# LouisBearing/BirdSoundClassif

Hardware: AMD Instinct MI355X
Metric: clips/sec (3 s @ 22.05 kHz) detect fwd (higher is better)
Workload: dtype f32; 1 GPU; BASELINE.json configs[1]: 1xMI355X inference, batch=64 synthetic 3 s clips (PCM16 @22.05 kHz resident in HBM) through the HIP STFT front end + detector forward + device post-processing, detections returned to the host; batch_per_gpu=64, distinct_clips=64, lanes=2

## Files before the change

birdsoundclassif_amd/_lib.py:

```python
import ctypes as C
import os
import subprocess

_HERE = os.path.dirname(os.path.abspath(__file__))
LIB_PATH = os.environ.get('NBM_LIB') or os.path.join(_HERE, 'libnbm_hip.so')
CSRC = os.path.join(_HERE, 'csrc')

_lib = None


class GemmDesc(C.Structure):
    _fields_ = [('x', C.c_void_p), ('w', C.c_void_p), ('y', C.c_void_p),
                ('scale', C.c_void_p), ('shift', C.c_void_p), ('residual', C.c_void_p),
                ('x_gs', C.c_int64), ('w_gs', C.c_int64), ('y_gs', C.c_int64), ('res_gs', C.c_int64),
                ('groups', C.c_int),
                ('B', C.c_int), ('H', C.c_int), ('W', C.c_int), ('Cin', C.c_int),
                ('N', C.c_int),
                ('kh', C.c_int), ('kw', C.c_int), ('stride', C.c_int), ('pad', C.c_int),
                ('Ho', C.c_int), ('Wo', C.c_int),
                ('x_ld', C.c_int), ('w_ld', C.c_int), ('y_ld', C.c_int), ('res_ld', C.c_int),
                ('alpha', C.c_float), ('act', C.c_int), ('shift_per_row', C.c_int),
                ('up', C.c_void_p), ('up_H', C.c_int), ('up_W', C.c_int),
                ('rows', C.c_void_p), ('rows_blocks', C.c_void_p),
                ('rows_mode', C.c_int), ('rows_count', C.c_int), ('rows_TH', C.c_int), ('rows_TW', C.c_int),
# ... 110 lines not shown
    'nbm_zero_tiles': [_P, _I, _I, _I, _I, _P, _I, _P, _P],
    'nbm_tiles_gather': [_P, _I, _I, _I, _I, _P, _I, _P, _P, _P],
    'nbm_tiles_scatter_add': [_P, _I, _I, _I, _I, _P, _I, _P, _P, _P],
    'nbm_proposal_iou': [_P, _P, _P, _I, _I, _I, _P, _P, _P],
    'nbm_anchor_targets': [_P, _I, _P, _P, _I, _I, _F, _F, _P, _P, _P, _P],
    'nbm_maxpool3x3s2_bwd': [_P, _P, _P, _I, _I, _I, _I, _I, _I, _P, _P, _P],
    'nbm_upsample_bilinear_bwd': [_P, _I, _I, _I, _I, _P, _I, _I, _I, _P],
    'nbm_tiles_upsample_bilinear_bwd_add': [_P, _I, _I, _I, _I, _P, _I, _P, _P, _I, _I, _P],
    'nbm_png_unfilter_gray8': [_P, _L, _I, _I, _I, _P, _L, _P, _P],
    'nbm_image_half_std_u8': [_P, _L, _I, _L, _P, _P],
    'nbm_randn_fill': [_U64, _L, _P, _P],
    'nbm_augment_batch': [_P, _P, _P, _I, _I, _I, _P, _P, _P, _P, _P, _P, _P],
    'nbm_u8_to_unit': [_P, _L, _P, _P],
    'nbm_wino_input': [_P, _I, _I, _I, _I, _P, _I, _P],
    'nbm_wino_output': [_P, _P, _P, _P, _I, _I, _I, _I, _I, _P, _I, _P, _P],
    'nbm_wino_outgrad': [_P, _I, _I, _I, _I, _P, _P, _I, _P],
    'nbm_wino_weight': [_P, _P, _I, _I, _I, _I, _P, _P],
    'nbm_wino_weight_grad': [_P, _P, _I, _I, _I, _P, _P],
    'nbm_wino23_rows': [_P, _I, _I, _I, _I, _P, _P],
    'nbm_wino23_conv_fused': [_P, _P, _P, _P, _P, _I, _I, _I, _I, _I, _I, _P, _I, _P],
    'nbm_wino23_rows_tiles': [_P, _I, _I, _I, _I, _P, _I, _P, _P, _P, _I, _P],
    'nbm_wino23_conv_fused_tiles': [_P, _P, _P, _P, _P, _I, _I, _I, _I, _I, _I, _P, _P, _I, _P, _P, _P],
    'nbm_roi_tiles': [_P, _P, _I, _I, _I, _I, _P, _P, _P, _I, _P, _P, _P],
    'nbm_wino23_input_tiles': [_P, _I, _I, _I, _I, _P, _I, _P, _P, _P],
    'nbm_wino23_outgrad_tiles': [_P, _I, _I, _I, _I, _P, _I, _P, _P, _P, _I, _P],
    'nbm_cell_outgrad': [_P, _I, _I, _I, _I, _I, _P, _P, _P],
    'nbm_cell_weight': [_P, _I, _I, _P, _I, _P, _I, _P],
    'nbm_cell_weight_fold': [_P, _P, _I, _I, _I, _I, _F, _P, _I, _P, _I, _P],
    'nbm_cell_weight_grad': [_P, _I, _I, _I, _P, _P],
    'nbm_cell_input': [_P, _I, _I, _I, _I, _I, _P, _I, _I, _P],
    'nbm_cell_input_up': [_P, _P, _I, _I, _I, _I, _I, _I, _I, _P, _I, _I, _P],
    'nbm_cell_patches': [_P, _I, _I, _I, _I, _I, _P, _I, _I, _P],
    'nbm_cell_patches_up': [_P, _P, _I, _I, _I, _I, _I, _I, _I, _P, _I, _I, _P],
    'nbm_cell_dgrad_output': [_P, _I, _I, _I, _I, _I, _P, _I, _I, _I, _P, _P],
    'nbm_cell_output': [_P, _P, _I, _I, _I, _I, _I, _P, _P],
    'nbm_weighted_sum': [_P, _P, _P, _P, _P, _L, _P],
    'nbm_weighted_sum_bwd': [_P, _P, _P, _P, _P, _P, _P, _P, _P, _L, _P],
    'nbm_softmax_rows_bwd': [_P, _P, _P, _L, _I, _F, _P],
    'nbm_pair_softmax_bwd': [_P, _P, _P, _L, _P],
    'nbm_dwconv3x3_bwd': [_P, _P, _P, _I, _I, _I, _I, _I, _I, _P, _P, _P, _I, _I, _P],
    'nbm_dwconv3x3_bwd_acc': [_P, _P, _I, _I, _I, _I, _I, _I, _P, _I, _I, _P],
    'nbm_film_fwd': [_P, _P, _P, _L, _I, _P],
    'nbm_film_bwd': [_P, _P, _P, _P, _P, _L, _I, _P],
    'nbm_bn_train_fwd': [_P, _L, _I, _P, _P, _F, _F, _P, _P, _P, _P, _P, _P, _P],
    'nbm_bn_train_bwd': [_P, _P, _L, _I, _P, _P, _P, _P, _P, _P, _P, _P],
    'nbm_roi_pool_bwd': [C.POINTER(C.c_void_p), C.POINTER(C.c_int), C.POINTER(C.c_int), _I, _I, _P, _P, _I, _I, _P, _P],
    'nbm_sqnorm_accum': [_P, _L, _P, _P],
    'nbm_adamw_step': [_P, _P, _P, _P, _L, _F, _F, _F, _F, _F, _I, _P, _F, _P],
}


def build(verbose=False):
    r = subprocess.run(['make', '-C', CSRC, '-j4'], capture_output=True, text=True)
    if verbose or r.returncode:
        print(r.stdout[-4000:], r.stderr[-4000:])
    if r.returncode:
        raise RuntimeError('building libnbm_hip.so failed')
    return LIB_PATH


def load():
    global _lib
    if _lib is not None:
        return _lib
    import torch
    if not os.path.isfile(LIB_PATH):
# ... 25 lines not shown
```

birdsoundclassif_amd/csrc/cellwino.hip:

```cpp
#include "nbm_common.h"

namespace {

constexpr int NP = 5;
constexpr int MAX_BIAS_N = 2048;
__device__ constexpr float CE[5][3] = {{1.f, 0.f, 0.f}, {1.f, 1.f, 1.f}, {1.f, -1.f, 1.f}, {1.f, 2.f, 4.f}, {1.f, -2.f, 4.f}};
__device__ constexpr float CV[5][5] = {{1.f, 0.f, 0.f, 0.f, 0.f},
                                       {0.f, 2.f / 3, -2.f / 3, -1.f / 12, 1.f / 12},
                                       {-5.f / 4, 2.f / 3, 2.f / 3, -1.f / 24, -1.f / 24},
                                       {0.f, -1.f / 6, 1.f / 6, 1.f / 12, -1.f / 12},
                                       {1.f / 4, -1.f / 6, -1.f / 6, 1.f / 24, 1.f / 24}};

struct CellGeom { int B, H, W, C4, S, OH, OW; long long T; };

__device__ __forceinline__ void cell_of(const CellGeom& q, unsigned cell, int& b, int& oy, int& ox) {
  ox = (int)(cell % (unsigned)q.OW);
  const unsigned r = cell / (unsigned)q.OW;
  oy = (int)(r % (unsigned)q.OH);
  b = (int)(r / (unsigned)q.OH);
}

__global__ __launch_bounds__(256) void cell_outgrad_kernel(const float* __restrict__ g, const CellGeom q, float* __restrict__ Vg,
                                                           float* __restrict__ bias_grad) {
  const f32x4* g4 = reinterpret_cast<const f32x4*>(g);
// ... 129 lines not shown
        lxs[l] = fminf(fmaxf(fx - x0, 0.f), 1.f);
        v00[l] = s4[((rb + y0) * Wc + x0) * q.C4 + c]; v01[l] = s4[((rb + y0) * Wc + x1i) * q.C4 + c];
        v10[l] = s4[((rb + y1) * Wc + x0) * q.C4 + c]; v11[l] = s4[((rb + y1) * Wc + x1i) * q.C4 + c];
      }
      __builtin_amdgcn_sched_barrier(0);
#pragma unroll
      for (int l = 0; l < NP; ++l) {
        const bool ok = yin && (unsigned)(q.S * ox - 2 + l) < (unsigned)q.W;
        const float lx = lxs[l], hx = 1.f - lx;
        f32x4 v;
#pragma unroll
        for (int e = 0; e < 4; ++e)
          v[e] = ok ? (hy * (hx * v00[l][e] + lx * v01[l][e]) + ly * (hx * v10[l][e] + lx * v11[l][e])) + bv[e] : 0.f;
        if constexpr (RAW) {
          v4[((long long)(j * NP + l) * q.T + cell) * ld4 + coff4 + c] = v;
        } else {
#pragma unroll
          for (int a = 0; a < NP; ++a)
            if (CV[j][a] != 0.f) t[a][l] += CV[j][a] * v;
        }
      }
    }
    if constexpr (RAW) continue;
#pragma unroll
    for (int a = 0; a < NP; ++a)
#pragma unroll
      for (int e = 0; e < NP; ++e) {
        f32x4 o = zero;
#pragma unroll
        for (int l = 0; l < NP; ++l)
          if (CV[l][e] != 0.f) o += CV[l][e] * t[a][l];
        v4[((long long)(a * NP + e) * q.T + cell) * ld4 + coff4 + c] = o;
      }
  }
}

__global__ __launch_bounds__(256) void cell_dgrad_output_kernel(const float* __restrict__ M, const CellGeom q, float* __restrict__ gx,
                                                                int cls, int ld4, int coff4, float* __restrict__ bias_grad) {
  const f32x4* m4 = reinterpret_cast<const f32x4*>(M);
  f32x4* o4 = reinterpret_cast<f32x4*>(gx);
  const f32x4 zero = {0.f, 0.f, 0.f, 0.f};
  f32x4 bsum = zero;
  int my_c = -1;
  const int cy = cls >= 0 ? cls >> 1 : 0, cx = cls >= 0 ? cls & 1 : 0;
  const int OHc = cls >= 0 ? (q.OH - cy + 1) >> 1 : q.OH, OWc = cls >= 0 ? (q.OW - cx + 1) >> 1 : q.OW;
  const unsigned total = (unsigned)((long long)q.B * OHc * OWc * q.C4);
  for (unsigned i = blockIdx.x * 256u + threadIdx.x; i < total; i += gridDim.x * 256u) {
    const int c = (int)(i % (unsigned)q.C4);
    unsigned rest = i / (unsigned)q.C4;
    int ox = (int)(rest % (unsigned)OWc); rest /= (unsigned)OWc;
    int oy = (int)(rest % (unsigned)OHc);
    const int b = (int)(rest / (unsigned)OHc);
    if (cls >= 0) { oy = 2 * oy + cy; ox = 2 * ox + cx; }
    const unsigned cell = ((unsigned)b * q.OH + oy) * q.OW + ox;
    my_c = c;
    f32x4 t[NP][NP];
#pragma unroll
    for (int j = 0; j < NP; ++j)
#pragma unroll
      for (int e = 0; e < NP; ++e) t[j][e] = zero;
#pragma unroll
    for (int a = 0; a < NP; ++a)
#pragma unroll
      for (int e = 0; e < NP; ++e) {
        const f32x4 v = m4[((long long)(a * NP + e) * q.T + cell) * ld4 + coff4 + c];
#pragma unroll
// ... 209 lines not shown
}

extern "C" int nbm_cell_input_up(const float* x1, const float* bias, int B, int H, int W, int C, int Hc, int Wc, int stride, float* Vx,
                                 int ld, int c_off, void* stream) {
  CellGeom q;
  if (!x1 || !Vx || !cell_geom(B, H, W, C, stride, q) || Hc <= 0 || Wc <= 0 || ld < c_off + C || c_off < 0) return NBM_EINVAL;
  if (!nbm_aligned16(x1) || !nbm_aligned16(Vx) || (bias && !nbm_aligned16(bias)) || (ld & 3) || (c_off & 3)) return NBM_EALIGN;
  const float sh = H > 1 ? (float)(Hc - 1) / (float)(H - 1) : 0.f, sw = W > 1 ? (float)(Wc - 1) / (float)(W - 1) : 0.f;
  hipLaunchKernelGGL(cell_input_up_kernel<false>, dim3(stream_grid(q.T * q.C4, q.C4)), dim3(256), 0, (hipStream_t)stream, x1, bias, q, Hc, Wc, sh,
                     sw, Vx, ld / 4, c_off / 4);
  return nbm_launch_status();
}

extern "C" int nbm_cell_patches(const float* x, int B, int H, int W, int C, int stride, float* Vx, int ld, int c_off, void* stream) {
  CellGeom q;
  if (!x || !Vx || !cell_geom(B, H, W, C, stride, q) || ld < c_off + C || c_off < 0) return NBM_EINVAL;
  if (!nbm_aligned16(x) || !nbm_aligned16(Vx) || (ld & 3) || (c_off & 3)) return NBM_EALIGN;
  hipLaunchKernelGGL(cell_input_kernel<true>, dim3(stream_grid(q.T * q.C4, q.C4)), dim3(256), 0, (hipStream_t)stream, x, q, Vx, ld / 4,
                     c_off / 4);
  return nbm_launch_status();
}

extern "C" int nbm_cell_patches_up(const float* x1, const float* bias, int B, int H, int W, int C, int Hc, int Wc, int stride, float* Vx,
                                   int ld, int c_off, void* stream) {
  CellGeom q;
  if (!x1 || !Vx || !cell_geom(B, H, W, C, stride, q) || Hc <= 0 || Wc <= 0 || ld < c_off + C || c_off < 0) return NBM_EINVAL;
  if (!nbm_aligned16(x1) || !nbm_aligned16(Vx) || (bias && !nbm_aligned16(bias)) || (ld & 3) || (c_off & 3)) return NBM_EALIGN;
  const float sh = H > 1 ? (float)(Hc - 1) / (float)(H - 1) : 0.f, sw = W > 1 ? (float)(Wc - 1) / (float)(W - 1) : 0.f;
  hipLaunchKernelGGL(cell_input_up_kernel<true>, dim3(stream_grid(q.T * q.C4, q.C4)), dim3(256), 0, (hipStream_t)stream, x1, bias, q, Hc, Wc,
                     sh, sw, Vx, ld / 4, c_off / 4);
  return nbm_launch_status();
}

extern "C" int nbm_cell_output(const float* M, const float* bias, int B, int H, int W, int N, int stride, float* y, void* stream) {
  CellGeom q;
  if (!M || !y || !cell_geom(B, H, W, N, stride, q)) return NBM_EINVAL;
  if (!nbm_aligned16(M) || !nbm_aligned16(y) || (bias && !nbm_aligned16(bias))) return NBM_EALIGN;
  hipLaunchKernelGGL(cell_output_kernel, dim3(stream_grid(q.T * q.C4, q.C4)), dim3(256), 0, (hipStream_t)stream, M, bias, q, y);
  return nbm_launch_status();
}

extern "C" int nbm_cell_dgrad_output(const float* M, int B, int H, int W, int C, int stride, float* gx, int parity_class, int ld,
                                     int c_off, float* bias_grad, void* stream) {
  CellGeom q;
  if (!M || !gx || parity_class > 3 || !cell_geom(B, H, W, C, stride, q, parity_class < 0 ? 5 : 3)) return NBM_EINVAL;
  if (ld < c_off + C || c_off < 0 || (ld & 3) || (c_off & 3) || (bias_grad && C > MAX_BIAS_N)) return NBM_EINVAL;
  if (!nbm_aligned16(M) || !nbm_aligned16(gx)) return NBM_EALIGN;
  hipLaunchKernelGGL(cell_dgrad_output_kernel, dim3(stream_grid(q.T * q.C4, q.C4)), dim3(256), 0, (hipStream_t)stream, M, q, gx,
                     parity_class, ld / 4, c_off / 4, bias_grad);
  return nbm_launch_status();
}

extern "C" int nbm_cell_weight(const float* w, int N, int C, float* U_nc, int ld, float* U_cn, int ldt, void* stream) {
  if (!w || (!U_nc && !U_cn) || N <= 0 || C <= 0 || (U_nc && ld < C) || (U_cn && ldt < C)) return NBM_EINVAL;
  hipLaunchKernelGGL(cell_weight_kernel, dim3((unsigned)((N * C + 255) / 256)), dim3(256), 0, (hipStream_t)stream, w, N, C, U_nc, ld, U_cn,
                     ldt);
  return nbm_launch_status();
}

extern "C" int nbm_cell_weight_fold(const float* w, const float* w_lat, int wl_ld, int N, int C, int Cin, float alpha, float* U_nc, int ld,
                                    float* U_cn, int ldt, void* stream) {
  if (!w || !w_lat || (!U_nc && !U_cn) || N <= 0 || C <= 0 || Cin <= 0 || wl_ld < Cin || (U_nc && ld < C + Cin) || (U_cn && ldt < C + Cin))
    return NBM_EINVAL;
  hipLaunchKernelGGL(cell_weight_fold_kernel, dim3((unsigned)((N * Cin + 255) / 256)), dim3(256), 0, (hipStream_t)stream, w, w_lat, wl_ld, N,
                     C, Cin, alpha, U_nc, ld, U_cn, ldt);
  return nbm_launch_status();
// ... 38 lines not shown
```

birdsoundclassif_amd/nets/_prep.py:

```python
import weakref

import torch
import torch.nn.functional as F

_cache = {}
_epoch = 0


def bump():
    global _epoch
    _epoch += 1


_DEBUG = __import__('os').environ.get('NBM_PREP_DEBUG') == '1'


def _evict(obj_id):
    for k in [k for k in _cache if k[0] == obj_id]:
        hit = _cache.pop(k, None)
        if _DEBUG and hit is not None:
            v = hit[2]
            ts = [t for t in (v if isinstance(v, (tuple, list)) else [v]) if torch.is_tensor(t)]
            print(f'_prep: evicted {k[1]} (key tensor died), values at {[hex(t.data_ptr()) for t in ts]}', flush=True)

# ... 128 lines not shown
    wp = pt_w.detach().double().reshape(pt_w.shape[0], m_)
    we = torch.einsum('nm,mcae->naec', wp, d)
    const = wp @ cb
    if lat_wk is not None:
        wl = lat_wk.detach().double()
        we = torch.cat([we, float(alpha) * torch.einsum('naec,ci->naei', we, wl)], -1)
    return we, const


def _rpn_extra(out_b, dw_w, dw_b, pt_w, scale, shift, lat_wk, alpha):
    others = [t for t in (out_b, dw_w, dw_b, pt_w, scale, shift, lat_wk) if t is not None]
    return tuple(v for t in others for v in (t.data_ptr(), t._version)) + (float(alpha),)


def rpn_composite(out_w, out_b, dw_w, dw_b, pt_w, scale, shift, lat_wk=None, alpha=1.0, parts=None):
    def make():
        we, const = _rpn_composite64(out_w, out_b, dw_w, dw_b, pt_w, 7, 7, lat_wk, alpha)
        rng = parts if parts is not None else ((0, we.shape[-1]),)
        ws = tuple(we[..., c0:c1].reshape(we.shape[0], -1).float().contiguous() for c0, c1 in rng)
        return ws, scale, (scale.double() * const + shift.double()).float().contiguous()
    return _cached(out_w, ('rpnc', lat_wk is not None, parts), make, extra=_rpn_extra(out_b, dw_w, dw_b, pt_w, scale, shift, lat_wk, alpha))


def rpn_composite_delta(out_w, out_b, dw_w, dw_b, pt_w, scale, shift, rmask, smask, taps, lat_wk=None, alpha=1.0):
    def make():
        we, const = _rpn_composite64(out_w, out_b, dw_w, dw_b, pt_w, rmask, smask, lat_wk, alpha)
        wi, ci = _rpn_composite64(out_w, out_b, dw_w, dw_b, pt_w, 7, 7, lat_wk, alpha)
        d = (we - wi).reshape(we.shape[0], 25, -1)[:, list(taps)] * scale.double()[:, None, None]
        return d.reshape(d.shape[0], -1).float().contiguous(), (scale.double() * (const - ci)).float().contiguous()
    return _cached(out_w, ('rpnd', int(rmask), int(smask), tuple(taps), lat_wk is not None), make,
                   extra=_rpn_extra(out_b, dw_w, dw_b, pt_w, scale, shift, lat_wk, alpha))


def lateral_of_projection(lat_w, lat_b, proj_w, proj_b):
    def make():
        wl = lat_w.detach().double().reshape(lat_w.shape[0], -1)
        wc = wl @ proj_w.detach().double()
        sh = wl @ proj_b.detach().double() + (lat_b.detach().double() if lat_b is not None else 0.0)
        return wc.float().contiguous(), sh.float().contiguous()
    others = [t for t in (lat_b, proj_w, proj_b) if t is not None]
    return _cached(lat_w, 'latproj', make, extra=tuple(v for t in others for v in (t.data_ptr(), t._version)))


def value_of_lateral(lat_w, proj_w, val_w, val_b):
    def make():
        wlo = lat_w.detach().double().reshape(lat_w.shape[0], -1) @ proj_w.detach().double()
        return (wlo @ val_w.detach().double()).float().contiguous(), (wlo @ val_b.detach().double()).float().contiguous()
    others = [proj_w, val_w, val_b]
    return _cached(lat_w, 'vallat', make, extra=tuple(v for t in others for v in (t.data_ptr(), t._version)))


def cat_rows(tag, *tensors):
    def make():
        return torch.cat([t.detach().reshape(t.shape[0], -1) if t.dim() > 1 else t.detach() for t in tensors], 0).contiguous()
    extra = tuple(v for t in tensors for v in (t.data_ptr(), t._version))
    return _cached(tensors[0], ('cat', tag), make, extra=extra)


def clear():
    _cache.clear()
```

birdsoundclassif_amd/ondemand.py:

```python
import ctypes as C
import os
import weakref
from typing import NamedTuple

import numpy as np
import torch

from . import ops
from .ops import check, lib, _ptr, _chk, _stream, gemm_conv, conv_wgrad

LAZY_FINEST = os.environ.get('NBM_LAZY_FINEST', '1') != '0'
COMPOSITE = os.environ.get('NBM_RPN_COMPOSITE', '1') != '0'
TRAIN_COMPOSITE = os.environ.get('NBM_RPN_COMPOSITE_TRAIN', '1') != '0'
LAT_CELL_BWD = os.environ.get('NBM_LAT_CELL_BWD', '1') != '0'
UPBWD_SPLIT = os.environ.get('NBM_UPBWD_SPLIT', '1') != '0'
ZERO_POOL = os.environ.get('NBM_ZERO_POOL', '1') != '0'
ZERO_POOL_CHECK = os.environ.get('NBM_ZERO_POOL_CHECK', '0') == '1'
LAZY_POISON = False
_LAZY = {}
_PATTERNS = {}
_ROI_TILE_BUF = {}


class TilePattern:
    __slots__ = ('tiles', 'blk_info', 'full', 'any', 'n', 'n_eff', 'frac', 'px_rows', 'n_px', 'entry_pm', 'tile_pm')


def wino23_pattern(B, H, W, stride, device, dilate=0):
    key = (B, H, W, stride, str(device), dilate)
    hit = _PATTERNS.get(key)
    if hit is None:
        TH, TW = (H + 1) // 2, (W + 1) // 2

        def need(n, nt):
            m = np.zeros(nt, dtype=np.int64)
            for o in range((n + 2 - 3) // stride + 1):
                for k in range(3):
                    for r in range(o * stride - 1 + k - dilate, o * stride - 1 + k + dilate + 1):
                        if 0 <= r < n:
                            m[r >> 1] |= 1 << (r & 1)
            return m
        ry, rx = need(H, TH), need(W, TW)
        planes_of = {0: 0, 1: 0b0111, 2: 0b1110, 3: 0b1111}

        def plane_mask(cy, cx):
# ... 315 lines not shown
    hit = _BORDER_IDX.get(key)
    if hit is None:
        rm, sm = _tap_masks(H, W, S)
        OH, OW = len(rm), len(sm)
        cls = {}
        for oy in range(OH):
            for ox in range(OW):
                if (rm[oy], sm[ox]) != (7, 7):
                    cls.setdefault((rm[oy], sm[ox]), []).append((oy, ox))
        hit = []
        for (r_, s_), cells in sorted(cls.items()):
            cells = sorted(cells)
            live_a = {a for oy, _ in cells for a in range(5) if 0 <= S * oy - 2 + a < H}
            live_e = {e for _, ox in cells for e in range(5) if 0 <= S * ox - 2 + e < W}
            dropped = [(r, c) for r in range(3) for c in range(3) if not ((r_ >> r) & 1 and (s_ >> c) & 1)]
            taps = [a * 5 + e for a in sorted(live_a) for e in sorted(live_e) if any(0 <= a - r <= 2 and 0 <= e - c <= 2 for r, c in dropped)]
            lin = np.array([oy * OW + ox for oy, ox in cells], dtype=np.int64)
            idx = (np.arange(nb, dtype=np.int64)[:, None] * (OH * OW) + lin[None, :]).reshape(-1)
            py = np.array([[S * oy - 2 + t // 5 for oy, _ in cells] for t in taps], dtype=np.int64)
            px = np.array([[S * ox - 2 + t % 5 for _, ox in cells] for t in taps], dtype=np.int64)
            pix = None
            if taps:
                inside = (py >= 0) & (py < H) & (px >= 0) & (px < W)
                one = np.clip(py, 0, H - 1) * W + np.clip(px, 0, W - 1)
                lin_px = (np.arange(nb, dtype=np.int64)[None, :, None] * (H * W) + one[:, None, :]).reshape(len(taps), -1)
                bad = None if bool(inside.all()) else torch.from_numpy(np.broadcast_to(~inside[:, None, :], (len(taps), nb, len(cells)))
                                                                       .reshape(len(taps), -1).copy()).to(device)
                pix = (torch.from_numpy(lin_px).to(device), bad)
            hit.append((r_, s_, tuple(taps), torch.tensor(taps, dtype=torch.int64, device=device)[:, None], torch.from_numpy(idx).to(device), pix))
        _BORDER_IDX[key] = hit
    return hit


def rpn_composite(fm, block):
    st = lazy_state(fm)
    if st is None or st.pending is None or st.raw is None:
        return None
    from .nets import _prep as prep
    S = st.stride
    if int(max(1, block.stride)) != S or block.stride < 1 or getattr(block, 'pe_proj', None) is not None:
        return None
    B, H, W, _ = fm.shape
    C_ = st.x.shape[-1]
    lt = st.lateral if st.lateral is not None and st.lateral.deferred else None
    Cin = lt.t.shape[-1] if lt is not None else 0
    K = C_ + Cin
    OH, OW = (H - 1) // S + 1, (W - 1) // S + 1
    out_w, out_b = st.raw
    scale, shift = prep.bn_affine(block.norm.weight, block.norm.bias, block.norm.running_mean, block.norm.running_var, block.norm.eps,
                                  conv_bias=block.pt_wise.bias)
    N2 = block.pt_wise.weight.shape[0]
    wargs = (out_w, out_b, block.depth_wise.weight, block.depth_wise.bias, block.pt_wise.weight, scale, shift)
    wkw = dict(lat_wk=lt.wk[:, :Cin] if lt is not None else None, alpha=lt.alpha if lt is not None else 1.0)
    if lt is not None:
        direct_t = Cin % 32 == 0
        operands = [('patch', 0, C_)] + ([('map', lt.t, 0, Cin, C_)] if direct_t else [])
        KV = C_ if direct_t else K
    elif C_ % 32 == 0:
        q32 = C_ // 32
        cc = C_ // (3 if q32 % 3 == 0 else 4 if q32 % 4 == 0 else 2 if q32 % 2 == 0 else 1)
        operands = [('map', st.x, c0, c0 + cc, c0) for c0 in range(0, C_, cc)]
        KV = 0
    else:
        operands, KV = [('patch', 0, C_)], C_
    parts = tuple((0, KV) if op[0] == 'patch' else (op[4], op[4] + op[3] - op[2]) for op in operands)
    ws, sc, sh = prep.rpn_composite(*wargs, **wkw, parts=parts)
    f = torch.empty((B, OH, OW, N2), device=fm.device, dtype=torch.float32)
    stream = _stream()
    keep_label, ops._PROFILE_LABEL = ops._PROFILE_LABEL, ('rpn-composite', H, W)
    try:
        for (b0, nb, pat) in st.chunks:
            T = nb * OH * OW
            V = None
            if KV:
                V = ops._wino_scratch(fm.device, 25 * T * KV, 0)[0]
                if lt is not None:
                    check(lib().nbm_cell_patches_up(_ptr(lt.up[b0:b0 + nb]), _ptr(lt.bias), nb, H, W, C_, lt.up.shape[1], lt.up.shape[2], S,
                                                    _ptr(V), KV, 0, stream), 'nbm_cell_patches_up')
                    if KV > C_:
                        check(lib().nbm_cell_patches(_ptr(lt.t[b0:b0 + nb]), nb, H, W, Cin, S, _ptr(V), KV, C_, stream), 'nbm_cell_patches')
                else:
                    check(lib().nbm_cell_patches(_ptr(st.x[b0:b0 + nb]), nb, H, W, C_, S, _ptr(V), KV, 0, stream), 'nbm_cell_patches')
            fc = f[b0:b0 + nb]
            border = _border_classes(nb, H, W, S, fm.device)
            R = None
            if border:
                R = torch.zeros((T, N2), device=fm.device, dtype=torch.float32)
                Vv = V[:25 * T * KV].view(25, T, KV) if KV else None
                for rmask, smask, taps, tap_idx, idx, pix in border:
                    if not taps:
                        continue
                    dwt, dsh = prep.rpn_composite_delta(*wargs, rmask, smask, taps, **wkw)
                    Tb, nt = idx.numel(), len(taps)
                    cols = []
                    for op in operands:
                        if op[0] == 'patch':
                            cols.append(Vv[tap_idx, idx[None, :]])
                        else:
                            m_ = op[1][b0:b0 + nb]
                            g_ = m_.reshape(-1, m_.shape[-1]).index_select(0, pix[0].reshape(-1))[:, op[2]:op[3]].reshape(nt, Tb, -1)
                            if pix[1] is not None:
                                g_ = g_.masked_fill(pix[1][..., None], 0.0)
                            cols.append(g_)
                    Vb = cols[0] if len(cols) == 1 else torch.cat(cols, -1)
                    fb = torch.empty((Tb, N2), device=fm.device, dtype=torch.float32)
                    if N2 % 32 == 0:
                        gemm_conv(Vb, dwt, fb, B=1, H=nt, W=Tb, Cin=K, N=32, kh=nt, kw=1, Ho=1, Wo=Tb, x_ld=K, w_ld=nt * K, y_ld=N2,
                                  groups=N2 // 32, x_gs=0, w_gs=32 * nt * K, y_gs=32, residual=dsh.expand(Tb, N2).contiguous(), res_ld=N2,
                                  res_gs=32)
                    else:
                        gemm_conv(Vb, dwt, fb, B=1, H=nt, W=Tb, Cin=K, N=N2, kh=nt, kw=1, Ho=1, Wo=Tb, x_ld=K, w_ld=nt * K, shift=dsh)
                    R.index_copy_(0, idx, fb)
            links = []
            for op, w in zip(operands, ws):
                if op[0] == 'patch':
                    ppl = max(1, min(5, ((1 << 31) - (1 << 24)) // (T * KV * 4)))
                    for p0 in range(0, 25, ppl):
                        npl = min(ppl, 25 - p0)
                        links.append(dict(x=V[p0 * T * KV:], w=w[:, p0 * KV:], B=1, H=npl, W=T, Cin=KV, kh=npl, kw=1, Ho=1, Wo=T, x_ld=KV,
                                          w_ld=25 * KV))
                else:
                    m_ = op[1][b0:b0 + nb]
                    cw = op[3] - op[2]
                    links.append(dict(x=m_[..., op[2]:], w=w, B=nb, H=H, W=W, Cin=cw, kh=5, kw=5, stride=S, pad=2, Ho=OH, Wo=OW,
                                      x_ld=m_.shape[-1], w_ld=25 * cw))
            for i, ln in enumerate(links):
                res = R if i == 0 else fc
                ops._PROFILE_LABEL = ('rpn-composite' if ln['kw'] == 1 else 'rpn-composite-map', H, W)
                gemm_conv(ln.pop('x'), ln.pop('w'), fc, N=N2, scale=sc, shift=sh if i == 0 else None, residual=res,
                          res_ld=N2 if res is not None else None, act=ops.ACT_SILU if i == len(links) - 1 else ops.ACT_NONE, **ln)
    finally:
        ops._PROFILE_LABEL = keep_label
    return f


_CE = ((1.0, 0.0, 0.0), (1.0, 1.0, 1.0), (1.0, -1.0, 1.0), (1.0, 2.0, 4.0), (1.0, -2.0, 4.0))


_DEV_CONST = {}


def _dev_const(device, key, values):
    k = (str(device), key)
    t = _DEV_CONST.get(k)
    if t is None:
        t = _DEV_CONST[k] = torch.tensor(values, dtype=torch.float32).to(device)
    return t


def _compose_rpn_cell(dw_w, dw_b, pt_w, pt_b, out_b, masks, mult):
    m_ = dw_w.shape[0]
    n1, n2 = m_ // mult, pt_w.shape[0]
    dev = dw_w.device
    E = _dev_const(dev, 'E', _CE)
    mr = _dev_const(dev, ('rmask', masks), [[float((rm >> r) & 1) for r in range(3)] for rm, _ in masks])
    ms = _dev_const(dev, ('smask', masks), [[float((sm >> c) & 1) for c in range(3)] for _, sm in masks])
    dw = dw_w.reshape(1, m_, 3, 3)
    pt = pt_w.reshape(n2, n1, mult)
    dwm = dw * mr[:, None, :, None] * ms[:, None, None, :]
    t = (E[None, None, :, :, None] * dwm[:, :, None, :, :]).sum(3)
    cw = (t[:, :, :, None, :] * E[None, None, None, :, :]).sum(4)
    cw = cw.reshape(len(masks), n1, mult, 25)
    A = (pt[None, None] * cw.permute(0, 3, 1, 2)[:, :, None]).sum(4)
# ... 596 lines not shown
```

include/nbm_hip.h:

```cpp
#ifndef NBM_HIP_H
#define NBM_HIP_H

#include <stdint.h>

#ifdef __cplusplus
extern "C" {
#endif

#define NBM_OK 0
#define NBM_EINVAL (-1)
#define NBM_EALIGN (-2)
#define NBM_EUNSUPPORTED (-3)

#define NBM_ACT_NONE 0
#define NBM_ACT_RELU 1
#define NBM_ACT_SILU 2
#define NBM_ACT_LEAKY 3

const char* nbm_version(void);

int nbm_graph_census(void* graph, long long counts[6]);

typedef struct nbm_gemm_desc {
  const float* x;
// ... 68 lines not shown
int nbm_wino_weight(const float* g, const float* scale, int N, int C, int transposed, int m, float* U, void* stream);
int nbm_wino_weight_grad(const float* dU, const float* row_scale, int N, int C, int m, float* dW, void* stream);

int nbm_wino23_rows(const float* x, int B, int H, int W, int C, float* R, void* stream);
int nbm_wino23_conv_fused(const float* R, const float* U, const float* scale, const float* shift, const float* mask,
                          int relu, int B, int H, int W, int C, int N, float* y, int variant, void* stream);

int nbm_wino23_rows_tiles(const float* x, int B, int H, int W, int C, const int* tiles, int n_entries, const int* n_blocks,
                          const unsigned* blk_info, float* R,
                          int skip_pattern_stride ,
                          void* stream);
int nbm_wino23_conv_fused_tiles(const float* R, const float* U, const float* scale, const float* shift, const float* mask,
                                int relu ,
                                int B, int H, int W, int C, int N, float* y, const int* tiles, int n_entries,
                                const int* n_blocks, const unsigned* blk_info, void* stream);
int nbm_roi_tiles(const float* rois, const int* n_roi, int B, int roi_cap, int n_levels, int level, const int* fh,
                  const int* fw, const unsigned char* skip, int dilate, int* tiles, int* n_blocks, void* stream);
int nbm_wino23_input_tiles(const float* x, int B, int H, int W, int C, const int* tiles, int n_list, const unsigned* plane_mask,
                           float* V, void* stream);
int nbm_wino23_outgrad_tiles(const float* g, int B, int H, int W, int N, const int* tiles, int n_list, const unsigned* plane_mask,
                             float* dM, float* bias_grad, int skip_pattern_stride, void* stream);
int nbm_cell_outgrad(const float* g, int B, int H, int W, int N, int stride, float* Vg, float* bias_grad, void* stream);
int nbm_cell_weight(const float* w, int N, int C, float* U_nc, int ld, float* U_cn, int ldt, void* stream);
int nbm_cell_weight_fold(const float* w, const float* w_lat, int wl_ld, int N, int C, int Cin, float alpha, float* U_nc, int ld,
                         float* U_cn, int ldt, void* stream);
int nbm_cell_weight_grad(const float* dU, int N, int C, int ld, float* dW, void* stream);
int nbm_cell_input(const float* x, int B, int H, int W, int C, int stride, float* Vx, int ld ,
                   int c_off , void* stream);
int nbm_cell_input_up(const float* x1, const float* bias, int B, int H, int W, int C, int Hc, int Wc, int stride, float* Vx, int ld,
                      int c_off, void* stream);
int nbm_cell_patches(const float* x, int B, int H, int W, int C, int stride, float* Vx, int ld, int c_off, void* stream);
int nbm_cell_patches_up(const float* x1, const float* bias, int B, int H, int W, int C, int Hc, int Wc, int stride, float* Vx, int ld,
                        int c_off, void* stream);

int nbm_copy_rect(float* strided, float* packed, int64_t n_outer, int64_t outer_pitch, int n_rows, int64_t row_pitch, int64_t width,
                  int to_strided, int zero_strided, void* stream);
int nbm_cell_dgrad_output(const float* M, int B, int H, int W, int C, int stride, float* gx, int parity_class,
                          int ld , int c_off ,
                          float* bias_grad , void* stream);
int nbm_cell_output(const float* M, const float* bias, int B, int H, int W, int N, int stride, float* y, void* stream);


int nbm_pcm16_to_wave(const int16_t* pcm, int64_t pcm_ld, int batch, int n, int upsample,
                      const int32_t* hq, int64_t first, int64_t count, float* out, int64_t out_ld, int lead,
                      int pad_mode, void* stream);

int nbm_resample_to_wave(const float* x, int64_t x_ld, int batch, int64_t n, int L, int M, const double* taps, int T,
                         int64_t first, int64_t count, float* out, int64_t out_ld, int lead, int pad_mode, int quant16,
                         void* stream);

#define NBM_WAV_MAX_CHANNELS 8
int nbm_wav_decode(const void* raw, int64_t raw_pitch, int batch, int tag, int bits, int channels, int64_t n, float* out,
                   int64_t out_pitch, void* stream);

int nbm_minmax_init(uint32_t* minmax, int batch, void* stream);
int nbm_stft_db(const float* wave, int64_t wave_ld, int batch, int n_frames, int hop, int n_fft,
                const double* basis, int basis_bin_tiles, int basis_ksteps, int n_bins, float floor_amp,
                float* db, int64_t db_bs, int db_ld, uint32_t* minmax, void* stream);

int nbm_spec_windows(const float* db, int64_t db_bs, int db_ld, int batch, int n_bins, int n_frames,
                     const uint32_t* minmax, float* img, int n_img, int w_pix, int hop_img,
                     const int32_t* last_cols, void* stream);

typedef struct nbm_window_entry {
  const float* db;
  const uint32_t* minmax;
// ... 220 lines not shown
```

Measured before the change: 1073 clips/s.

## Fold horizontal bilinear upsample into RPN composite weights per output column

Adds a column-folded path for the RPN composite conv on upsampled lateral features. The horizontal bilinear interpolation is folded into per-output-column weights, so the new kernel only interpolates vertically and gathers 4 source columns instead of 5 interpolated taps, and the GEMM runs grouped per column with K=5*4*C. This is meant to cut patch-expansion memory traffic and GEMM depth, at the cost of per-column weight tensors (cached), more border-handling code and extra grouped GEMM launches for border rows.

```diff
diff --git a/birdsoundclassif_amd/_lib.py b/birdsoundclassif_amd/_lib.py
--- a/birdsoundclassif_amd/_lib.py
+++ b/birdsoundclassif_amd/_lib.py
@@ -166,6 +166,7 @@
     'nbm_cell_input_up': [_P, _P, _I, _I, _I, _I, _I, _I, _I, _P, _I, _I, _P],
     'nbm_cell_patches': [_P, _I, _I, _I, _I, _I, _P, _I, _I, _P],
     'nbm_cell_patches_up': [_P, _P, _I, _I, _I, _I, _I, _I, _I, _P, _I, _I, _P],
+    'nbm_cell_patches_up_cols': [_P, _P, _I, _I, _I, _I, _I, _I, _I, _P, _P],
     'nbm_cell_dgrad_output': [_P, _I, _I, _I, _I, _I, _P, _I, _I, _I, _P, _P],
     'nbm_cell_output': [_P, _P, _I, _I, _I, _I, _I, _P, _P],
     'nbm_weighted_sum': [_P, _P, _P, _P, _P, _L, _P],
diff --git a/birdsoundclassif_amd/csrc/cellwino.hip b/birdsoundclassif_amd/csrc/cellwino.hip
--- a/birdsoundclassif_amd/csrc/cellwino.hip
+++ b/birdsoundclassif_amd/csrc/cellwino.hip
@@ -185,6 +185,72 @@
           if (CV[l][e] != 0.f) o += CV[l][e] * t[a][l];
         v4[((long long)(a * NP + e) * q.T + cell) * ld4 + coff4 + c] = o;
       }
+  }
+}
+
+__host__ __device__ inline int cell_col_window(int ox, int S, int W, int Wc, float sw, unsigned& used) {
+#pragma clang fp contract(off)
+  int xb = 0x7fffffff, x0s[NP];
+  for (int l = 0; l < NP; ++l) {
+    const int xx = S * ox - 2 + l;
+    const int xc = xx < 0 ? 0 : (xx > W - 1 ? W - 1 : xx);
+    const float fx = sw * xc;
+    x0s[l] = (int)fx;
+    if ((unsigned)xx < (unsigned)W && x0s[l] < xb) xb = x0s[l];
+  }
+  used = 0u;
+  for (int l = 0; l < NP; ++l)
+    if ((unsigned)(S * ox - 2 + l) < (unsigned)W) {
+      const int d0 = x0s[l] - xb, d1 = d0 + (x0s[l] < Wc - 1 ? 1 : 0);
+      used |= (1u << (d0 < 31 ? d0 : 31)) | (1u << (d1 < 31 ? d1 : 31));
+    }
+  return xb;
+}
+
+__global__ __launch_bounds__(256) void cell_patches_up_cols_kernel(const float* __restrict__ x1, const float* __restrict__ bias,
+                                                                   const CellGeom q, int Hc, int Wc, float sh, float sw,
+                                                                   float* __restrict__ Vx) {
+#pragma clang fp contract(off)
+  constexpr int NS = 4;
+  const f32x4* s4 = reinterpret_cast<const f32x4*>(x1);
+  f32x4* v4 = reinterpret_cast<f32x4*>(Vx);
+  const f32x4 zero = {0.f, 0.f, 0.f, 0.f};
+  const unsigned total = (unsigned)(q.T * q.C4);
+  const long long rows = (long long)q.B * q.OH;
+  for (unsigned i = blockIdx.x * 256u + threadIdx.x; i < total; i += gridDim.x * 256u) {
+    const int c = (int)(i % (unsigned)q.C4);
+    const unsigned cell = i / (unsigned)q.C4;
+    int b, oy, ox;
+    cell_of(q, cell, b, oy, ox);
+    const f32x4 bv = bias ? reinterpret_cast<const f32x4*>(bias)[c] : zero;
+    unsigned used;
+    const int xb = cell_col_window(ox, q.S, q.W, Wc, sw, used);
+    const long long rb = (long long)b * Hc;
+    const long long out0 = ((long long)ox * (NP * NS) * rows + (long long)b * q.OH + oy) * q.C4 + c;
+#pragma unroll
+    for (int j = 0; j < NP; ++j) {
+      const int y = q.S * oy - 2 + j;
+      const bool yin = (unsigned)y < (unsigned)q.H;
+      const float fy = sh * (yin ? y : 0);
+      const int y0 = (int)fy, y1 = y0 + (y0 < Hc - 1 ? 1 : 0);
+      const float ly = fminf(fmaxf(fy - y0, 0.f), 1.f), hy = 1.f - ly;
+      f32x4 v0[NS], v1[NS];
+#pragma unroll
+      for (int s = 0; s < NS; ++s) {
+        const int xs = min(xb + s, Wc - 1);
+        v0[s] = s4[((rb + y0) * Wc + xs) * q.C4 + c];
+        v1[s] = s4[((rb + y1) * Wc + xs) * q.C4 + c];
+      }
+      __builtin_amdgcn_sched_barrier(0);
+#pragma unroll
+      for (int s = 0; s < NS; ++s) {
+        const bool ok = yin && ((used >> s) & 1u);
+        f32x4 v;
+#pragma unroll
+        for (int e = 0; e < 4; ++e) v[e] = ok ? (hy * v0[s][e] + ly * v1[s][e]) + bv[e] : 0.f;
+        v4[out0 + (long long)(j * NS + s) * rows * q.C4] = v;
+      }
+    }
   }
 }
 
@@ -460,6 +526,22 @@
   return nbm_launch_status();
 }
 
+extern "C" int nbm_cell_patches_up_cols(const float* x1, const float* bias, int B, int H, int W, int C, int Hc, int Wc, int stride, float* Vx,
+                                        void* stream) {
+  CellGeom q;
+  if (!x1 || !Vx || !cell_geom(B, H, W, C, stride, q) || Hc <= 0 || Wc <= 0) return NBM_EINVAL;
+  if (!nbm_aligned16(x1) || !nbm_aligned16(Vx) || (bias && !nbm_aligned16(bias))) return NBM_EALIGN;
+  const float sh = H > 1 ? (float)(Hc - 1) / (float)(H - 1) : 0.f, sw = W > 1 ? (float)(Wc - 1) / (float)(W - 1) : 0.f;
+  for (int ox = 0; ox < q.OW; ++ox) {
+    unsigned used;
+    cell_col_window(ox, stride, W, Wc, sw, used);
+    if (used >> 4) return NBM_EUNSUPPORTED;
+  }
+  hipLaunchKernelGGL(cell_patches_up_cols_kernel, dim3(stream_grid(q.T * q.C4, q.C4)), dim3(256), 0, (hipStream_t)stream, x1, bias, q, Hc,
+                     Wc, sh, sw, Vx);
+  return nbm_launch_status();
+}
+
 extern "C" int nbm_cell_output(const float* M, const float* bias, int B, int H, int W, int N, int stride, float* y, void* stream) {
   CellGeom q;
   if (!M || !y || !cell_geom(B, H, W, N, stride, q)) return NBM_EINVAL;
diff --git a/birdsoundclassif_amd/nets/_prep.py b/birdsoundclassif_amd/nets/_prep.py
--- a/birdsoundclassif_amd/nets/_prep.py
+++ b/birdsoundclassif_amd/nets/_prep.py
@@ -184,6 +184,83 @@
                    extra=_rpn_extra(out_b, dw_w, dw_b, pt_w, scale, shift, lat_wk, alpha))
 
 
+XFOLD_COLS = 4
+_XFOLD_GEOM = {}
+
+
+def xfold_columns(W, Wc, S):
+    import numpy as np
+    key = (int(W), int(Wc), int(S))
+    if key not in _XFOLD_GEOM:
+        OW = (W - 1) // S + 1
+        f32 = np.float32
+        sw = f32(Wc - 1) / f32(W - 1) if W > 1 else f32(0.0)
+        x = S * np.arange(OW)[:, None] - 2 + np.arange(5)[None, :]
+        inside = (x >= 0) & (x < W)
+        fx = sw * np.clip(x, 0, W - 1).astype(f32)
+        assert fx.dtype == np.float32
+        x0 = fx.astype(np.int64)
+        x1 = x0 + (x0 < Wc - 1)
+        lx = np.minimum(np.maximum(fx - x0.astype(f32), f32(0.0)), f32(1.0))
+        hx = f32(1.0) - lx
+        xbase = np.where(inside, x0, np.iinfo(np.int64).max).min(1)
+        hit = None
+        if int(np.where(inside, x1 - xbase[:, None], 0).max()) < XFOLD_COLS:
+            cx = np.zeros((OW, 5, XFOLD_COLS), dtype=np.float64)
+            used = np.zeros((OW, XFOLD_COLS), dtype=bool)
+            for ox in range(OW):
+                for l in range(5):
+                    if inside[ox, l]:
+                        cx[ox, l, x0[ox, l] - xbase[ox]] += float(hx[ox, l])
+                        cx[ox, l, x1[ox, l] - xbase[ox]] += float(lx[ox, l])
+                        used[ox, x0[ox, l] - xbase[ox]] = used[ox, x1[ox, l] - xbase[ox]] = True
+            hit = (xbase, used, cx)
+        _XFOLD_GEOM[key] = hit
+    return _XFOLD_GEOM[key]
+
+
+def xfold64(we, cx):
+    return torch.einsum('gls,nrlc->gnrsc', cx, we)
+
+
+def rpn_composite_xfold(out_w, out_b, dw_w, dw_b, pt_w, scale, shift, W, Wc, S, smasks, rows=None, lat_wk=None, alpha=1.0):
+    geom = xfold_columns(W, Wc, S)
+    if geom is None:
+        return None
+    smasks = tuple(int(s) for s in smasks)
+    c = out_w.shape[1]
+
+    def make():
+        cx = torch.from_numpy(geom[2]).to(out_w.device)
+        n = pt_w.shape[0]
+        a_rows = list(range(5)) if rows is None else list(rows[1])
+        out = torch.empty((len(smasks), n, len(a_rows), XFOLD_COLS * c), dtype=torch.float32, device=out_w.device)
+        for sm in sorted(set(smasks)):
+            we = _rpn_composite64(out_w, out_b, dw_w, dw_b, pt_w, 7, sm, lat_wk, alpha)[0][..., :c]
+            if rows is not None:
+                we = (_rpn_composite64(out_w, out_b, dw_w, dw_b, pt_w, rows[0], sm, lat_wk, alpha)[0][..., :c] - we) * \
+                    scale.double()[:, None, None, None]
+            we = we[:, a_rows]
+            oxs = [ox for ox, s in enumerate(smasks) if s == sm]
+            for i in range(0, len(oxs), 8):
+                sel = torch.tensor(oxs[i:i + 8], device=out_w.device)
+                out[sel] = xfold64(we, cx[sel]).reshape(len(sel), n, len(a_rows), -1).float()
+        if rows is None:
+            return out.reshape(len(smasks), n, -1)
+        return out.permute(2, 0, 1, 3).contiguous()
+    tag = ('rpnxf', int(W), int(Wc), int(S), smasks, None if rows is None else (int(rows[0]), tuple(rows[1])), lat_wk is not None)
+    return _cached(out_w, tag, make, extra=_rpn_extra(out_b, dw_w, dw_b, pt_w, scale, shift, lat_wk, alpha))
+
+
+def rpn_composite_delta_part(out_w, out_b, dw_w, dw_b, pt_w, scale, shift, rmask, smask, taps, c0, c1, lat_wk=None, alpha=1.0):
+    def make():
+        d, dsh = rpn_composite_delta(out_w, out_b, dw_w, dw_b, pt_w, scale, shift, rmask, smask, taps, lat_wk=lat_wk, alpha=alpha)
+        d = d.reshape(d.shape[0], len(taps), -1)[:, :, c0:c1]
+        return d.reshape(d.shape[0], -1).contiguous(), dsh
+    return _cached(out_w, ('rpndp', int(rmask), int(smask), tuple(taps), int(c0), int(c1), lat_wk is not None), make,
+                   extra=_rpn_extra(out_b, dw_w, dw_b, pt_w, scale, shift, lat_wk, alpha))
+
+
 def lateral_of_projection(lat_w, lat_b, proj_w, proj_b):
     def make():
         wl = lat_w.detach().double().reshape(lat_w.shape[0], -1)
diff --git a/birdsoundclassif_amd/ondemand.py b/birdsoundclassif_amd/ondemand.py
--- a/birdsoundclassif_amd/ondemand.py
+++ b/birdsoundclassif_amd/ondemand.py
@@ -11,6 +11,8 @@
 
 LAZY_FINEST = os.environ.get('NBM_LAZY_FINEST', '1') != '0'
 COMPOSITE = os.environ.get('NBM_RPN_COMPOSITE', '1') != '0'
+XFOLD = os.environ.get('NBM_RPN_XFOLD', '1') != '0'
+XFOLD_CALLS = [0]
 TRAIN_COMPOSITE = os.environ.get('NBM_RPN_COMPOSITE_TRAIN', '1') != '0'
 LAT_CELL_BWD = os.environ.get('NBM_LAT_CELL_BWD', '1') != '0'
 UPBWD_SPLIT = os.environ.get('NBM_UPBWD_SPLIT', '1') != '0'
@@ -392,6 +394,10 @@
     return hit
 
 
+def _xfold_applies(nb, OH, OW, C_):
+    return 4 * nb * OH * C_ * 4 < (1 << 31) - (1 << 24)
+
+
 def rpn_composite(fm, block):
     st = lazy_state(fm)
     if st is None or st.pending is None or st.raw is None:
@@ -427,12 +433,24 @@
     ws, sc, sh = prep.rpn_composite(*wargs, **wkw, parts=parts)
     f = torch.empty((B, OH, OW, N2), device=fm.device, dtype=torch.float32)
     stream = _stream()
+    xfold_ok = bool(XFOLD and lt is not None and direct_t and C_ % 32 == 0 and N2 % 4 == 0 and
+                    prep.xfold_columns(W, lt.up.shape[2], S) is not None)
+    rmasks, smasks = _tap_masks(H, W, S)
     keep_label, ops._PROFILE_LABEL = ops._PROFILE_LABEL, ('rpn-composite', H, W)
     try:
         for (b0, nb, pat) in st.chunks:
             T = nb * OH * OW
             V = None
-            if KV:
+            fold = xfold_ok and _xfold_applies(nb, OH, OW, C_)
+            if fold:
+                XFOLD_CALLS[0] += 1
+                NC = prep.XFOLD_COLS
+                rows_g = nb * OH
+                V = ops._wino_scratch(fm.device, 5 * NC * T * C_, 0)[0]
+                check(lib().nbm_cell_patches_up_cols(_ptr(lt.up[b0:b0 + nb]), _ptr(lt.bias), nb, H, W, C_, lt.up.shape[1], lt.up.shape[2], S,
+                                                     _ptr(V), stream), 'nbm_cell_patches_up_cols')
+                wf = prep.rpn_composite_xfold(*wargs, W, lt.up.shape[2], S, smasks, **wkw)
+            elif KV:
                 V = ops._wino_scratch(fm.device, 25 * T * KV, 0)[0]
                 if lt is not None:
                     check(lib().nbm_cell_patches_up(_ptr(lt.up[b0:b0 + nb]), _ptr(lt.bias), nb, H, W, C_, lt.up.shape[1], lt.up.shape[2], S,
@@ -446,14 +464,19 @@
             R = None
             if border:
                 R = torch.zeros((T, N2), device=fm.device, dtype=torch.float32)
-                Vv = V[:25 * T * KV].view(25, T, KV) if KV else None
+                Vv = V[:25 * T * KV].view(25, T, KV) if KV and not fold else None
+                b_ops = [op for op in operands if not (fold and op[0] == 'patch')]
+                Kb = K - C_ if fold else K
                 for rmask, smask, taps, tap_idx, idx, pix in border:
                     if not taps:
                         continue
-                    dwt, dsh = prep.rpn_composite_delta(*wargs, rmask, smask, taps, **wkw)
+                    if fold:
+                        dwt, dsh = prep.rpn_composite_delta_part(*wargs, rmask, smask, taps, C_, K, **wkw)
+                    else:
+                        dwt, dsh = prep.rpn_composite_delta(*wargs, rmask, smask, taps, **wkw)
                     Tb, nt = idx.numel(), len(taps)
                     cols = []
-                    for op in operands:
+                    for op in b_ops:
                         if op[0] == 'patch':
                             cols.append(Vv[tap_idx, idx[None, :]])
                         else:
@@ -465,15 +488,33 @@
                     Vb = cols[0] if len(cols) == 1 else torch.cat(cols, -1)
                     fb = torch.empty((Tb, N2), device=fm.device, dtype=torch.float32)
                     if N2 % 32 == 0:
-                        gemm_conv(Vb, dwt, fb, B=1, H=nt, W=Tb, Cin=K, N=32, kh=nt, kw=1, Ho=1, Wo=Tb, x_ld=K, w_ld=nt * K, y_ld=N2,
-                                  groups=N2 // 32, x_gs=0, w_gs=32 * nt * K, y_gs=32, residual=dsh.expand(Tb, N2).contiguous(), res_ld=N2,
+                        gemm_conv(Vb, dwt, fb, B=1, H=nt, W=Tb, Cin=Kb, N=32, kh=nt, kw=1, Ho=1, Wo=Tb, x_ld=Kb, w_ld=nt * Kb, y_ld=N2,
+                                  groups=N2 // 32, x_gs=0, w_gs=32 * nt * Kb, y_gs=32, residual=dsh.expand(Tb, N2).contiguous(), res_ld=N2,
                                   res_gs=32)
                     else:
-                        gemm_conv(Vb, dwt, fb, B=1, H=nt, W=Tb, Cin=K, N=N2, kh=nt, kw=1, Ho=1, Wo=Tb, x_ld=K, w_ld=nt * K, shift=dsh)
+                        gemm_conv(Vb, dwt, fb, B=1, H=nt, W=Tb, Cin=Kb, N=N2, kh=nt, kw=1, Ho=1, Wo=Tb, x_ld=Kb, w_ld=nt * Kb, shift=dsh)
                     R.index_copy_(0, idx, fb)
+                if fold:
+                    for oy in range(OH):
+                        if rmasks[oy] == 7:
+                            continue
+                        a_rows = tuple(a for a in range(5) if 0 <= S * oy - 2 + a < H and
+                                       any(0 <= a - r <= 2 for r in range(3) if not (rmasks[oy] >> r) & 1))
+                        dwf = prep.rpn_composite_xfold(*wargs, W, lt.up.shape[2], S, smasks, rows=(rmasks[oy], a_rows), **wkw)
+                        Ro = R[oy * OW:]
+                        ops._PROFILE_LABEL = ('rpn-composite', H, W, 'cols')
+                        for i, a in enumerate(a_rows):
+                            gemm_conv(V[(a * NC * rows_g + oy) * C_:], dwf[i], Ro, B=1, H=NC, W=nb, Cin=C_, N=N2, kh=NC, kw=1, Ho=1, Wo=nb,
+                                      x_ld=OH * C_, w_ld=NC * C_, y_ld=OH * OW * N2, groups=OW, x_gs=5 * NC * rows_g * C_,
+                                      w_gs=N2 * NC * C_, y_gs=N2, residual=Ro, res_ld=OH * OW * N2, res_gs=N2)
             links = []
             for op, w in zip(operands, ws):
-                if op[0] == 'patch':
+                if op[0] == 'patch' and fold:
+                    for j in range(5):
+                        links.append(dict(x=V[j * NC * rows_g * C_:], w=wf[:, :, j * NC * C_:], B=1, H=NC, W=rows_g, Cin=C_, kh=NC, kw=1, Ho=1,
+                                          Wo=rows_g, x_ld=C_, w_ld=5 * NC * C_, groups=OW, x_gs=5 * NC * rows_g * C_, w_gs=N2 * 5 * NC * C_,
+                                          y_gs=N2, y_ld=OW * N2, res_gs=N2, res_ld=OW * N2))
+                elif op[0] == 'patch':
                     ppl = max(1, min(5, ((1 << 31) - (1 << 24)) // (T * KV * 4)))
                     for p0 in range(0, 25, ppl):
                         npl = min(ppl, 25 - p0)
@@ -486,9 +527,10 @@
                                       x_ld=m_.shape[-1], w_ld=25 * cw))
             for i, ln in enumerate(links):
                 res = R if i == 0 else fc
-                ops._PROFILE_LABEL = ('rpn-composite' if ln['kw'] == 1 else 'rpn-composite-map', H, W)
+                ops._PROFILE_LABEL = ('rpn-composite' if ln['kw'] == 1 else 'rpn-composite-map', H, W) + (('cols',) if 'groups' in ln else ())
+                res_ld = ln.pop('res_ld', N2)
                 gemm_conv(ln.pop('x'), ln.pop('w'), fc, N=N2, scale=sc, shift=sh if i == 0 else None, residual=res,
-                          res_ld=N2 if res is not None else None, act=ops.ACT_SILU if i == len(links) - 1 else ops.ACT_NONE, **ln)
+                          res_ld=res_ld if res is not None else None, act=ops.ACT_SILU if i == len(links) - 1 else ops.ACT_NONE, **ln)
     finally:
         ops._PROFILE_LABEL = keep_label
     return f
diff --git a/include/nbm_hip.h b/include/nbm_hip.h
--- a/include/nbm_hip.h
+++ b/include/nbm_hip.h
@@ -124,6 +124,8 @@
 int nbm_cell_patches(const float* x, int B, int H, int W, int C, int stride, float* Vx, int ld, int c_off, void* stream);
 int nbm_cell_patches_up(const float* x1, const float* bias, int B, int H, int W, int C, int Hc, int Wc, int stride, float* Vx, int ld,
                         int c_off, void* stream);
+int nbm_cell_patches_up_cols(const float* x1, const float* bias, int B, int H, int W, int C, int Hc, int Wc, int stride, float* Vx,
+                             void* stream);
 
 int nbm_copy_rect(float* strided, float* packed, int64_t n_outer, int64_t outer_pitch, int n_rows, int64_t row_pitch, int64_t width,
                   int to_strided, int zero_strided, void* stream);
```

Measured after the change: 1090 clips/s, median of 6. +1.6%, better.
